# eniac/Reef

Hardware: AMD Instinct MI355X
Metric: msm_scalar_point_pairs_per_sec (higher is better)
Workload: dtype u32

## Files before the change

reef_amd/csrc/ec.h:

```cpp
#pragma once
#include "field.h"

#if defined(__HIP_DEVICE_COMPILE__)
#define REEF_ANY(x) __any(x)
#else
#define REEF_ANY(x) (x)
#endif

namespace reef {

struct affine {
    fe x, y;
};
struct xyzz {
    fe x, y, zz, zzz;
};
struct alignas(16) affine256 {
    fe256 x, y;
};
struct alignas(16) jacobian256 {
    fe256 x, y, z;
};
struct alignas(16) xyzz_mem {
    u32 w[36];
};

REEF_HD bool affine_is_inf(const affine &p) { return fe_is_literal_zero(p.x) && fe_is_literal_zero(p.y); }
template <int C> REEF_HD bool xyzz_is_inf(const xyzz &p) { return fe_is_zero<C>(p.zz); }

REEF_HD xyzz xyzz_identity() {
    xyzz r;
    r.x = fe_zero(); r.y = fe_zero(); r.zz = fe_zero(); r.zzz = fe_zero();
    return r;
}
REEF_HD xyzz xyzz_select(bool c, const xyzz &a, const xyzz &b) {
    xyzz r;
    r.x = fe_select(c, a.x, b.x); r.y = fe_select(c, a.y, b.y);
    r.zz = fe_select(c, a.zz, b.zz); r.zzz = fe_select(c, a.zzz, b.zzz);
    return r;
}
template <int C> REEF_HD xyzz xyzz_from_affine(const affine &p) {
    xyzz r;
    const bool inf = affine_is_inf(p);
    r.x = p.x; r.y = p.y;
    r.zz = fe_select(inf, fe_zero(), fe_one<C>());
    r.zzz = r.zz;
    return r;
}
template <int C> REEF_HD affine affine_neg(const affine &p) {
    affine r;
    r.x = p.x;
    r.y = fe_select(affine_is_inf(p), p.y, fe_neg<C, 2>(p.y));
    return r;
}
template <int C> REEF_HD xyzz xyzz_neg(const xyzz &p) {
    xyzz r = p;
    r.y = fe_neg<C, 4>(p.y);
    return r;
}

template <int C> REEF_HD xyzz xyzz_dbl_affine(const affine &p) {
    xyzz r;
    const fe u = fe_dbl<C>(p.y);
    const fe v = fe_sqr<C>(u);
    const fe w = fe_mul<C>(u, v);
    const fe s = fe_mul<C>(p.x, v);
    const fe xx = fe_sqr<C>(p.x);
    const fe m = fe_add<C>(fe_dbl<C>(xx), xx);
    r.x = fe_sub<C, 4>(fe_sqr<C>(m), fe_dbl<C>(s));
    r.y = fe_sub<C, 2>(fe_mul<C>(m, fe_sub<C, 8>(s, r.x)),
                       fe_mul<C>(w, p.y));
    r.zz = v;
    r.zzz = w;
    return r;
}

template <int C> REEF_HD xyzz xyzz_dbl(const xyzz &p) {
    xyzz r;
    const fe u = fe_dbl<C>(p.y);
    const fe v = fe_sqr<C>(u);
    const fe w = fe_mul<C>(u, v);
    const fe s = fe_mul<C>(p.x, v);
    const fe xx = fe_sqr<C>(p.x);
    const fe m = fe_add<C>(fe_dbl<C>(xx), xx);
    r.x = fe_sub<C, 4>(fe_sqr<C>(m), fe_dbl<C>(s));
    r.y = fe_sub<C, 2>(fe_mul<C>(m, fe_sub<C, 8>(s, r.x)),
                       fe_mul<C>(w, p.y));
    r.zz = fe_mul<C>(v, p.zz);
    r.zzz = fe_mul<C>(w, p.zzz);
    return r;
}

template <int C> REEF_HD xyzz xyzz_madd_flag(const xyzz &a, bool a_known_empty, const affine &p) {
    const bool a_inf = a_known_empty || xyzz_is_inf<C>(a);
    const bool p_inf = affine_is_inf(p);
    const fe pp_ = fe_mul_sub<C, 8>(p.x, a.zz, a.x);
    const fe rr = fe_mul_sub<C, 4>(p.y, a.zzz, a.y);
    xyzz r;
    if (__builtin_expect(fe_is_zero<C>(pp_) && fe_is_zero<C>(rr) && !a_inf && !p_inf, 0)) {
        r = xyzz_dbl_affine<C>(p);
    } else {
        const fe pp = fe_sqr<C>(pp_);
        const fe ppp = fe_mul<C>(pp_, pp);
        const fe q = fe_mul<C>(a.x, pp);
        fe t;
#pragma unroll
        for (int i = 0; i < 9; ++i) t.l[i] = ppp.l[i] + 2u * q.l[i];
        REEF_SET_BOUND(t, REEF_GET_BOUND(ppp) + 2.0 * REEF_GET_BOUND(q));
        r.x = fe_sqr_sub<C, 4>(rr, t);
        r.y = fe_mul2_add<C>(rr, fe_sub<C, 8>(q, r.x), fe_neg<C, 4>(a.y), ppp);
        r.zz = fe_mul<C>(a.zz, pp);
        r.zzz = fe_mul<C>(a.zzz, ppp);
    }
    if (REEF_ANY(a_inf)) {
        xyzz from_p;
        from_p.x = p.x; from_p.y = p.y; from_p.zz = fe_one<C>(); from_p.zzz = from_p.zz;
        r = xyzz_select(a_inf, from_p, r);
    }
    if (REEF_ANY(p_inf)) r = xyzz_select(p_inf, a, r);
    return r;
}

template <int C> REEF_HD xyzz xyzz_madd(const xyzz &a, const affine &p) { return xyzz_madd_flag<C>(a, false, p); }

template <int C> REEF_HD xyzz xyzz_add(const xyzz &a, const xyzz &b) {
    const bool a_inf = xyzz_is_inf<C>(a);
    const bool b_inf = xyzz_is_inf<C>(b);
    const fe u1 = fe_mul<C>(a.x, b.zz);
    const fe u2 = fe_mul<C>(b.x, a.zz);
    const fe s1 = fe_mul<C>(a.y, b.zzz);
    const fe s2 = fe_mul<C>(b.y, a.zzz);
    const fe pp_ = fe_sub<C, 2>(u2, u1);
    const fe rr = fe_sub<C, 2>(s2, s1);
    xyzz r;
    if (__builtin_expect(fe_is_zero<C>(pp_) && fe_is_zero<C>(rr) && !a_inf && !b_inf, 0)) {
        r = xyzz_dbl<C>(a);
    } else {
        const fe pp = fe_sqr<C>(pp_);
        const fe ppp = fe_mul<C>(pp_, pp);
        const fe q = fe_mul<C>(u1, pp);
        const fe t = fe_add<C>(ppp, fe_dbl<C>(q));
        r.x = fe_sub<C, 4>(fe_sqr<C>(rr), t);
        r.y = fe_mul2_add<C>(rr, fe_sub<C, 8>(q, r.x), fe_neg<C, 2>(s1), ppp);
        r.zz = fe_mul<C>(fe_mul<C>(a.zz, b.zz), pp);
        r.zzz = fe_mul<C>(fe_mul<C>(a.zzz, b.zzz), ppp);
    }
    r = xyzz_select(a_inf, b, r);
    r = xyzz_select(b_inf, a, r);
    return r;
}

REEF_HD affine affine_from_table(const affine256 &m) {
    affine r;
    r.x = fe_from_table(m.x);
    r.y = fe_from_table(m.y);
    return r;
}
template <int C> REEF_HD affine256 affine_to_table(const affine &p) {
    affine256 m;
    m.x = fe_to_table<C>(p.x);
    m.y = fe_to_table<C>(p.y);
    return m;
}
template <int C> REEF_HD affine affine_from_abi(const affine256 &m) {
    affine r;
    r.x = fe_from_abi<C>(m.x);
    r.y = fe_from_abi<C>(m.y);
    return r;
}
template <int C> REEF_HD affine256 affine_to_abi(const affine &p) {
    affine256 m;
    m.x = fe_to_abi<C>(p.x);
    m.y = fe_to_abi<C>(p.y);
    return m;
}
REEF_HD xyzz xyzz_from_mem(const xyzz_mem &m) {
    xyzz r;
#pragma unroll
    for (int i = 0; i < 9; ++i) {
        r.x.l[i] = m.w[i]; r.y.l[i] = m.w[9 + i]; r.zz.l[i] = m.w[18 + i]; r.zzz.l[i] = m.w[27 + i];
    }
    REEF_SET_BOUND(r.x, 6.0); REEF_SET_BOUND(r.y, 3.6); REEF_SET_BOUND(r.zz, 1.6); REEF_SET_BOUND(r.zzz, 1.6);
    return r;
}
REEF_HD xyzz_mem xyzz_to_mem(const xyzz &p) {
    xyzz_mem m;
#if defined(REEF_BOUNDS)
    if (p.x.bound > 6.0 || p.y.bound > 3.6 || p.zz.bound > 1.6 || p.zzz.bound > 1.6) REEF_BOUND_FAIL("xyzz_to_mem: invariant");
#endif
#pragma unroll
    for (int i = 0; i < 9; ++i) {
        m.w[i] = p.x.l[i]; m.w[9 + i] = p.y.l[i]; m.w[18 + i] = p.zz.l[i]; m.w[27 + i] = p.zzz.l[i];
    }
    return m;
}

template <int C> REEF_HD jacobian256 xyzz_to_abi_jacobian(const xyzz &p) {
    jacobian256 r;
    const bool inf = xyzz_is_inf<C>(p);
    r.x = fe_to_abi<C>(fe_select(inf, fe_zero(), fe_mul<C>(p.x, p.zz)));
    r.y = fe_to_abi<C>(fe_select(inf, fe_zero(), fe_mul<C>(p.y, p.zzz)));
    r.z = fe_to_abi<C>(fe_select(inf, fe_zero(), p.zz));
    return r;
}
template <int C> REEF_HD xyzz xyzz_from_abi_jacobian(const jacobian256 &m) {
    xyzz r;
    const fe z = fe_from_abi<C>(m.z);
    r.x = fe_from_abi<C>(m.x);
    r.y = fe_from_abi<C>(m.y);
    r.zz = fe_sqr<C>(z);
    r.zzz = fe_mul<C>(r.zz, z);
    return r;
}

template <int C> REEF_HD affine xyzz_to_affine_with_inv(const xyzz &p, const fe &t) {
    affine r;
    const bool inf = xyzz_is_inf<C>(p);
    const fe izz = fe_mul<C>(t, p.zzz);
    const fe izzz = fe_mul<C>(t, p.zz);
    r.x = fe_select(inf, fe_zero(), fe_mul<C>(p.x, izz));
    r.y = fe_select(inf, fe_zero(), fe_mul<C>(p.y, izzz));
    return r;
}
template <int C> REEF_HD affine xyzz_to_affine(const xyzz &p) {
    return xyzz_to_affine_with_inv<C>(p, fe_inv<C>(fe_mul<C>(p.zz, p.zzz)));
}

template <int C> REEF_HD fe256 affine_compress(const affine &p) {
    fe one = fe_zero();
    one.l[0] = 1;
    REEF_SET_BOUND(one, 1.0);
    fe256 x = fe_pack(fe_canon<C>(fe_mul<C>(p.x, one)));
    const fe y = fe_canon<C>(fe_mul<C>(p.y, one));
    x.w[7] |= (y.l[0] & 1u) << 31;
    if (affine_is_inf(p)) {
#pragma unroll
        for (int i = 0; i < 8; ++i) x.w[i] = 0;
    }
    return x;
}

template <int C> REEF_HD xyzz xyzz_scalar_mul(const affine &p, const u32 *k, int top_bit) {
    xyzz acc = xyzz_identity();
    for (int i = top_bit; i >= 0; --i) {
        acc = xyzz_dbl<C>(acc);
        if ((k[i >> 5] >> (i & 31)) & 1u) acc = xyzz_madd<C>(acc, p);
    }
    return acc;
}

}
```

reef_amd/csrc/field.h:

```cpp
#pragma once
#include <stdint.h>

#if defined(__HIPCC__)
#include <hip/hip_runtime.h>
#define REEF_HD __host__ __device__ __forceinline__
#else
#define REEF_HD inline
#endif

namespace reef {
typedef uint32_t u32;
typedef uint64_t u64;
typedef int64_t i64;
#if defined(__HIPCC__)
#if defined(REEF_VEC_VARIANT) && REEF_VEC_VARIANT == 2
typedef u32 u32x2 __attribute__((ext_vector_type(2), may_alias));
typedef u32 u32x4 __attribute__((ext_vector_type(4), may_alias));
REEF_HD u32x2 mk_u32x2(u32 a, u32 b) { u32x2 v; v.x = a; v.y = b; return v; }
REEF_HD u32x4 mk_u32x4(u32 a, u32 b, u32 c, u32 d) { u32x4 v; v.x = a; v.y = b; v.z = c; v.w = d; return v; }
#else
typedef uint2 u32x2;
typedef uint4 u32x4;
REEF_HD u32x2 mk_u32x2(u32 a, u32 b) { return make_uint2(a, b); }
REEF_HD u32x4 mk_u32x4(u32 a, u32 b, u32 c, u32 d) { return make_uint4(a, b, c, d); }
#endif
#endif
}

#include "field_consts.h"

#if defined(REEF_BOUNDS)
#include <assert.h>
#include <stdio.h>
#include <stdlib.h>
#define REEF_BOUND_FAIL(msg) do { fprintf(stderr, "REEF_BOUNDS violation: %s (%s:%d)\n", msg, __FILE__, __LINE__); abort(); } while (0)
#endif

namespace reef {

static constexpr u32 LIMB_BITS = 29;
static constexpr u32 LIMB_MASK = (1u << LIMB_BITS) - 1u;

struct fe {
    u32 l[9];
#if defined(REEF_BOUNDS)
    double bound;
#endif
};

struct alignas(16) fe256 {
    u32 w[8];
};

#if defined(REEF_BOUNDS)
#define REEF_SET_BOUND(x, b) ((x).bound = (b))
#define REEF_GET_BOUND(x) ((x).bound)
#else
#define REEF_SET_BOUND(x, b) ((void)0)
#define REEF_GET_BOUND(x) (0.0)
#endif

REEF_HD fe fe_zero() {
    fe r;
#pragma unroll
    for (int i = 0; i < 9; ++i) r.l[i] = 0;
    REEF_SET_BOUND(r, 0.0);
    return r;
}
template <int F> REEF_HD fe fe_const(const u32 (&c)[9], double bound) {
    fe r;
#pragma unroll
    for (int i = 0; i < 9; ++i) r.l[i] = c[i];
    REEF_SET_BOUND(r, bound);
    (void)bound;
    return r;
}
template <int F> REEF_HD fe fe_one() { return fe_const<F>(FC<F>::ONE, 1.0); }

REEF_HD fe fe_select(bool c, const fe &a, const fe &b) {
    fe r;
#pragma unroll
    for (int i = 0; i < 9; ++i) r.l[i] = c ? a.l[i] : b.l[i];
#if defined(REEF_BOUNDS)
    r.bound = a.bound > b.bound ? a.bound : b.bound;
#endif
    return r;
}

REEF_HD fe fe_norm(const fe &a) {
    fe r;
    r.l[0] = a.l[0] & LIMB_MASK;
#pragma unroll
    for (int i = 1; i < 8; ++i) r.l[i] = (a.l[i] & LIMB_MASK) + (a.l[i - 1] >> LIMB_BITS);
    r.l[8] = a.l[8] + (a.l[7] >> LIMB_BITS);
#if defined(REEF_BOUNDS)
    r.bound = a.bound;
    if ((u64)a.l[8] + (a.l[7] >> LIMB_BITS) >= (1ull << 29)) REEF_BOUND_FAIL("top limb overflow in fe_norm");
#endif
    return r;
}

REEF_HD fe fe_norm_strict(const fe &a) {
    fe r;
    u32 c = 0;
#pragma unroll
    for (int i = 0; i < 8; ++i) {
        u32 t = a.l[i] + c;
        r.l[i] = t & LIMB_MASK;
        c = t >> LIMB_BITS;
    }
    r.l[8] = a.l[8] + c;
#if defined(REEF_BOUNDS)
    r.bound = a.bound;
#endif
    return r;
}

template <int F> REEF_HD fe fe_add(const fe &a, const fe &b) {
    fe s;
#pragma unroll
    for (int i = 0; i < 9; ++i) s.l[i] = a.l[i] + b.l[i];
    REEF_SET_BOUND(s, REEF_GET_BOUND(a) + REEF_GET_BOUND(b));
    return fe_norm(s);
}
template <int F> REEF_HD fe fe_dbl(const fe &a) { return fe_add<F>(a, a); }

template <int F, int K> REEF_HD const u32 (&fe_bias())[9] {
    static_assert(K == 2 || K == 4 || K == 8 || K == 16 || K == 32, "bias");
    if constexpr (K == 2) return FC<F>::BIAS2;
    else if constexpr (K == 4) return FC<F>::BIAS4;
    else if constexpr (K == 8) return FC<F>::BIAS8;
    else if constexpr (K == 16) return FC<F>::BIAS16;
    else return FC<F>::BIAS32;
}

template <int F, int K> REEF_HD fe fe_sub(const fe &a, const fe &b) {
    fe d;
#pragma unroll
    for (int i = 0; i < 9; ++i) d.l[i] = a.l[i] + fe_bias<F, K>()[i] - b.l[i];
#if defined(REEF_BOUNDS)
    if (b.bound > (double)K * (1.0 - 1e-5)) REEF_BOUND_FAIL("fe_sub: subtrahend bound exceeds the bias");
    for (int i = 0; i < 9; ++i) {
        i64 t = (i64)a.l[i] + (i64)fe_bias<F, K>()[i] - (i64)b.l[i];
        if (t < 0 || t >= (1ll << 32)) REEF_BOUND_FAIL("fe_sub: limb out of range");
    }
    d.bound = a.bound + K;
#endif
    return fe_norm(d);
}
template <int F, int K> REEF_HD fe fe_neg(const fe &a) { return fe_sub<F, K>(fe_zero(), a); }

#if defined(__HIP_DEVICE_COMPILE__)
__device__ __forceinline__ void mad_acc_1(u64 &acc, u32 a) {
    u64 sink;
    asm("v_mad_u64_u32 %0, %1, %2, 1, %0" : "+v"(acc), "=&s"(sink) : "v"(a));
}
#else
REEF_HD void mad_acc_1(u64 &acc, u32 a) { acc += a; }
#endif

#if !defined(__HIP_DEVICE_COMPILE__)
REEF_HD void mad_row_new(u64 (&t)[10], const u32 (&a)[9], u32 b, u64 bias) {
    for (int j = 0; j < 9; ++j) t[j] = (u64)a[j] * b + bias;
}
REEF_HD void mad_row_acc(u64 (&t)[10], const u32 (&a)[9], u32 b) {
    for (int j = 0; j < 8; ++j) t[j] += (u64)a[j] * b;
    t[8] = (u64)a[8] * b;
}
REEF_HD void mad_row_add(u64 (&t)[10], const u32 (&a)[9], u32 b) {
    for (int j = 0; j < 9; ++j) t[j] += (u64)a[j] * b;
}
REEF_HD void mad_reduce(u64 (&t)[10], u32 q, u32 m1, u32 m2, u32 m3, u32 m4, u32 top) {
    t[1] += (u64)q * m1; t[2] += (u64)q * m2; t[3] += (u64)q * m3; t[4] += (u64)q * m4;
    t[8] += (u64)q * top;
}
template <int I> REEF_HD void sqr_row(u64 (&t)[10], const u32 (&a)[9], const u32 (&a2)[9], u64 bias) {
    if (I == 0) {
        t[0] = (u64)a[0] * a[0] + bias;
        for (int j = 1; j < 9; ++j) t[j] = (u64)a[0] * a2[j] + bias;
    } else if (I == 8) {
        t[8] = (u64)a[8] * a[8];
    } else {
        t[I] += (u64)a[I] * a[I];
        for (int j = I + 1; j < 8; ++j) t[j] += (u64)a[I] * a2[j];
        t[8] = (u64)a[I] * a2[8];
    }
}
#else
}
#include "field_mad_gfx950.h"
namespace reef {
template <int I> __device__ __forceinline__ void sqr_row(u64 (&t)[10], const u32 (&a)[9], const u32 (&a2)[9], u64 bias) {
    if constexpr (I == 0) sqr_row0(t, a, a2, bias);
    else if constexpr (I == 1) sqr_row1(t, a, a2);
    else if constexpr (I == 2) sqr_row2(t, a, a2);
    else if constexpr (I == 3) sqr_row3(t, a, a2);
    else if constexpr (I == 4) sqr_row4(t, a, a2);
    else if constexpr (I == 5) sqr_row5(t, a, a2);
    else if constexpr (I == 6) sqr_row6(t, a, a2);
    else if constexpr (I == 7) sqr_row7(t, a, a2);
    else sqr_row8(t, a, a2);
    (void)bias;
}
#endif

static constexpr u64 MONT_BIAS = LIMB_MASK;
REEF_HD void mont_bias(u64 (&t)[10]) {
#pragma unroll
    for (int j = 0; j < 9; ++j) t[j] += MONT_BIAS;
}

template <int F> REEF_HD void mont_round(u64 (&t)[10]) {
    const u32 q = ~(u32)t[0] & LIMB_MASK;
    mad_reduce(t, q, FC<F>::M1, FC<F>::M2, FC<F>::M3, FC<F>::M4, 1u << 22);
    t[1] += t[0] >> LIMB_BITS;
#pragma unroll
    for (int j = 0; j < 9; ++j) t[j] = t[j + 1];
}

template <int F> REEF_HD fe mont_finish(const u64 (&t)[10]) {
    fe r;
    u64 c = 0;
#pragma unroll
    for (int i = 0; i < 8; ++i) {
        const u64 v = t[i] + c;
        r.l[i] = (u32)v & LIMB_MASK;
        c = v >> LIMB_BITS;
    }
    r.l[8] = (u32)(t[8] + c);
#if defined(REEF_BOUNDS)
    if (t[8] + c >= (1ull << 29)) REEF_BOUND_FAIL("Montgomery product: result top limb overflow");
#endif
    return r;
}

template <int F> REEF_HD fe fe_mul(const fe &a, const fe &b) {
#if defined(REEF_BOUNDS)
    if (a.bound * b.bound >= 128.0) REEF_BOUND_FAIL("fe_mul: (A/M)(B/M) >= 128");
    for (int i = 0; i < 8; ++i)
        if (a.l[i] > LIMB_MASK + 8 || b.l[i] > LIMB_MASK + 8) REEF_BOUND_FAIL("fe_mul: operand not normalised");
#endif
    u64 t[10];
    t[9] = 0;
    mad_row_new(t, a.l, b.l[0], MONT_BIAS);
    mont_round<F>(t);
#pragma unroll
    for (int i = 1; i < 9; ++i) {
        mad_row_acc(t, a.l, b.l[i]);
        mont_round<F>(t);
    }
    fe r = mont_finish<F>(t);
    REEF_SET_BOUND(r, 1.0 + REEF_GET_BOUND(a) * REEF_GET_BOUND(b) / 128.0);
    return r;
}

template <int F> REEF_HD fe fe_mul2_add(const fe &a, const fe &b, const fe &c, const fe &d) {
#if defined(REEF_BOUNDS)
    if (a.bound * b.bound + c.bound * d.bound >= 128.0) REEF_BOUND_FAIL("fe_mul2_add: (A/M)(B/M) + (C/M)(D/M) >= 128");
    for (int i = 0; i < 8; ++i)
        if (a.l[i] > LIMB_MASK + 8 || b.l[i] > LIMB_MASK + 8 || c.l[i] > LIMB_MASK + 8 || d.l[i] > LIMB_MASK + 8)
            REEF_BOUND_FAIL("fe_mul2_add: operand not normalised");
#endif
    u64 t[10];
    t[9] = 0;
    mad_row_new(t, a.l, b.l[0], MONT_BIAS);
    mad_row_add(t, c.l, d.l[0]);
    mont_round<F>(t);
#pragma unroll
    for (int i = 1; i < 9; ++i) {
        mad_row_acc(t, a.l, b.l[i]);
        mad_row_add(t, c.l, d.l[i]);
        mont_round<F>(t);
    }
    fe r = mont_finish<F>(t);
    REEF_SET_BOUND(r, 1.0 + (REEF_GET_BOUND(a) * REEF_GET_BOUND(b) + REEF_GET_BOUND(c) * REEF_GET_BOUND(d)) / 128.0);
    return r;
}

template <int F, int K> REEF_HD fe fe_mul_sub(const fe &a, const fe &b, const fe &c) {
#if defined(REEF_BOUNDS)
    if (a.bound * b.bound >= 128.0) REEF_BOUND_FAIL("fe_mul_sub: (A/M)(B/M) >= 128");
    if (c.bound > (double)K * (1.0 - 1e-5)) REEF_BOUND_FAIL("fe_mul_sub: subtrahend bound exceeds the bias");
    for (int i = 0; i < 8; ++i)
        if (a.l[i] > LIMB_MASK + 8 || b.l[i] > LIMB_MASK + 8) REEF_BOUND_FAIL("fe_mul_sub: operand not normalised");
    for (int i = 0; i < 9; ++i)
        if (c.l[i] > fe_bias<F, K>()[i]) REEF_BOUND_FAIL("fe_mul_sub: subtrahend limb exceeds the bias limb");
#endif
    u64 t[10];
    t[9] = 0;
    mad_row_new(t, a.l, b.l[0], MONT_BIAS);
    mont_round<F>(t);
#pragma unroll
    for (int i = 1; i < 9; ++i) {
        mad_row_acc(t, a.l, b.l[i]);
        mont_round<F>(t);
    }
#pragma unroll
    for (int i = 0; i < 9; ++i) mad_acc_1(t[i], fe_bias<F, K>()[i] - c.l[i]);
    fe r = mont_finish<F>(t);
    REEF_SET_BOUND(r, 1.0 + REEF_GET_BOUND(a) * REEF_GET_BOUND(b) / 128.0 + K);
    return r;
}

template <int F> REEF_HD fe fe_sqr(const fe &a) {
#if defined(REEF_BOUNDS)
    if (a.bound * a.bound >= 128.0) REEF_BOUND_FAIL("fe_sqr: (A/M)^2 >= 128");
    for (int i = 0; i < 8; ++i)
        if (a.l[i] > LIMB_MASK + 8) REEF_BOUND_FAIL("fe_sqr: operand not normalised");
#endif
    u32 a2[9];
#pragma unroll
    for (int i = 0; i < 9; ++i) a2[i] = a.l[i] << 1;
    u64 t[10];
    t[9] = 0;
    sqr_row<0>(t, a.l, a2, MONT_BIAS); mont_round<F>(t);
    sqr_row<1>(t, a.l, a2, MONT_BIAS); mont_round<F>(t);
    sqr_row<2>(t, a.l, a2, MONT_BIAS); mont_round<F>(t);
    sqr_row<3>(t, a.l, a2, MONT_BIAS); mont_round<F>(t);
    sqr_row<4>(t, a.l, a2, MONT_BIAS); mont_round<F>(t);
    sqr_row<5>(t, a.l, a2, MONT_BIAS); mont_round<F>(t);
    sqr_row<6>(t, a.l, a2, MONT_BIAS); mont_round<F>(t);
    sqr_row<7>(t, a.l, a2, MONT_BIAS); mont_round<F>(t);
    sqr_row<8>(t, a.l, a2, MONT_BIAS); mont_round<F>(t);
    fe r = mont_finish<F>(t);
    REEF_SET_BOUND(r, 1.0 + REEF_GET_BOUND(a) * REEF_GET_BOUND(a) / 128.0);
    return r;
}

template <int F, int K> REEF_HD fe fe_sqr_sub(const fe &a, const fe &c) {
#if defined(REEF_BOUNDS)
    if (a.bound * a.bound >= 128.0) REEF_BOUND_FAIL("fe_sqr_sub: (A/M)^2 >= 128");
    if (c.bound > (double)K * (1.0 - 1e-5)) REEF_BOUND_FAIL("fe_sqr_sub: subtrahend bound exceeds the bias");
    for (int i = 0; i < 8; ++i)
        if (a.l[i] > LIMB_MASK + 8) REEF_BOUND_FAIL("fe_sqr_sub: operand not normalised");
    for (int i = 0; i < 9; ++i)
        if (c.l[i] > fe_bias<F, K>()[i]) REEF_BOUND_FAIL("fe_sqr_sub: subtrahend limb exceeds the bias limb");
#endif
    u32 a2[9];
#pragma unroll
    for (int i = 0; i < 9; ++i) a2[i] = a.l[i] << 1;
    u64 t[10];
    t[9] = 0;
    sqr_row<0>(t, a.l, a2, MONT_BIAS); mont_round<F>(t);
    sqr_row<1>(t, a.l, a2, MONT_BIAS); mont_round<F>(t);
    sqr_row<2>(t, a.l, a2, MONT_BIAS); mont_round<F>(t);
    sqr_row<3>(t, a.l, a2, MONT_BIAS); mont_round<F>(t);
    sqr_row<4>(t, a.l, a2, MONT_BIAS); mont_round<F>(t);
    sqr_row<5>(t, a.l, a2, MONT_BIAS); mont_round<F>(t);
    sqr_row<6>(t, a.l, a2, MONT_BIAS); mont_round<F>(t);
    sqr_row<7>(t, a.l, a2, MONT_BIAS); mont_round<F>(t);
    sqr_row<8>(t, a.l, a2, MONT_BIAS); mont_round<F>(t);
#pragma unroll
    for (int i = 0; i < 9; ++i) mad_acc_1(t[i], fe_bias<F, K>()[i] - c.l[i]);
    fe r = mont_finish<F>(t);
    REEF_SET_BOUND(r, 1.0 + REEF_GET_BOUND(a) * REEF_GET_BOUND(a) / 128.0 + K);
    return r;
}

template <int F> REEF_HD fe fe_small_multiple(u32 j) {
    fe r;
    u64 c = 0;
#pragma unroll
    for (int i = 0; i < 8; ++i) {
        u64 v = (u64)j * FC<F>::MOD[i] + c;
        r.l[i] = (u32)v & LIMB_MASK;
        c = v >> LIMB_BITS;
    }
    r.l[8] = (u32)((u64)j * FC<F>::MOD[8] + c);
    REEF_SET_BOUND(r, (double)j);
    return r;
}

template <int F> REEF_HD bool fe_is_zero(const fe &a) {
#if defined(REEF_BOUNDS)
    if (a.bound >= 64.0) REEF_BOUND_FAIL("fe_is_zero: bound >= 64");
#endif
    const u32 j = a.l[0];
    if (__builtin_expect(j >= 64u, 1)) return false;
    const fe s = fe_norm_strict(a);
    const fe m = fe_small_multiple<F>(j);
    u32 d = 0;
#pragma unroll
    for (int i = 0; i < 9; ++i) d |= s.l[i] ^ m.l[i];
    return d == 0;
}
REEF_HD bool fe_is_literal_zero(const fe &a) {
    u32 d = 0;
#pragma unroll
    for (int i = 0; i < 9; ++i) d |= a.l[i];
    return d == 0;
}

template <int F> REEF_HD fe fe_canon(const fe &a) {
    const fe s = fe_norm_strict(a);
    const u32 q = s.l[8] >> 22;
    fe r;
    i64 c = 0;
#pragma unroll
    for (int i = 0; i < 8; ++i) {
        i64 v = (i64)s.l[i] - (i64)((u64)q * FC<F>::MOD[i]) + c;
        r.l[i] = (u32)v & LIMB_MASK;
        c = v >> LIMB_BITS;
    }
    i64 top = (i64)s.l[8] - (i64)((u64)q * FC<F>::MOD[8]) + c;
    const bool neg = top < 0;
    u32 cc = 0;
#pragma unroll
    for (int i = 0; i < 8; ++i) {
        u32 v = r.l[i] + (neg ? FC<F>::MOD[i] : 0u) + cc;
        r.l[i] = v & LIMB_MASK;
        cc = v >> LIMB_BITS;
    }
    r.l[8] = (u32)(top + (neg ? (i64)FC<F>::MOD[8] : 0) + cc);
    REEF_SET_BOUND(r, 1.0);
    return r;
}

REEF_HD fe fe_unpack(const fe256 &p) {
    fe r;
#pragma unroll
    for (int i = 0; i < 9; ++i) {
        const int bit = 29 * i, w = bit >> 5, s = bit & 31;
        u32 v = p.w[w] >> s;
        if (s > 3 && w + 1 < 8) v |= p.w[w + 1] << (32 - s);
        r.l[i] = (i == 8) ? v : (v & LIMB_MASK);
    }
    REEF_SET_BOUND(r, 4.0);
    return r;
}
REEF_HD fe256 fe_pack(const fe &a) {
    fe256 p;
#pragma unroll
    for (int w = 0; w < 8; ++w) {
        const int bit = 32 * w, i = bit / 29, s = bit - 29 * i;
        u32 v = a.l[i] >> s;
        if (i + 1 < 9) v |= a.l[i + 1] << (29 - s);
        if (29 - s + 29 < 32 && i + 2 < 9) v |= a.l[i + 2] << (58 - s);
        p.w[w] = v;
    }
    return p;
}

template <int F> REEF_HD fe fe_from_abi(const fe256 &p) {
    fe x = fe_unpack(p);
    REEF_SET_BOUND(x, 1.0);
    return fe_mul<F>(x, fe_const<F>(FC<F>::C_IN, 1.0));
}
template <int F> REEF_HD fe256 fe_to_abi(const fe &a) {
    return fe_pack(fe_canon<F>(fe_mul<F>(a, fe_const<F>(FC<F>::C_OUT, 1.0))));
}
template <int F> REEF_HD fe256 fe_to_table(const fe &a) { return fe_pack(fe_canon<F>(a)); }
REEF_HD fe fe_from_table(const fe256 &p) {
    fe x = fe_unpack(p);
    REEF_SET_BOUND(x, 1.0);
    return x;
}
template <int F> REEF_HD fe256 fe_abi_to_integer(const fe256 &p) {
    fe x = fe_unpack(p);
    REEF_SET_BOUND(x, 1.0);
    fe c32 = fe_zero();
    c32.l[0] = 32;
    REEF_SET_BOUND(c32, 1.0);
    return fe_pack(fe_canon<F>(fe_mul<F>(x, c32)));
}
template <int F> REEF_HD fe fe_from_integer(const fe256 &p) {
    fe x = fe_unpack(p);
    REEF_SET_BOUND(x, 1.0);
    return fe_mul<F>(x, fe_const<F>(FC<F>::C_R2, 1.0));
}
template <int F> REEF_HD fe256 fe_to_integer(const fe &x) {
    fe one = fe_zero();
    one.l[0] = 1;
    REEF_SET_BOUND(one, 1.0);
    return fe_pack(fe_canon<F>(fe_mul<F>(x, one)));
}
template <int F> REEF_HD fe fe_from_caller(const fe256 &p, bool is_mont) { return is_mont ? fe_from_abi<F>(p) : fe_from_integer<F>(p); }
template <int F> REEF_HD fe256 fe_to_caller(const fe &x, bool to_mont) { return to_mont ? fe_to_abi<F>(x) : fe_to_integer<F>(x); }

template <int F> REEF_HD fe fe_inv(const fe &a) {
    u32 e[9];
#pragma unroll
    for (int i = 0; i < 9; ++i) e[i] = FC<F>::MOD[i];
    e[0] = LIMB_MASK;
    e[1] -= 1;
    fe acc = fe_one<F>();
    for (int i = 254; i >= 0; --i) {
        acc = fe_sqr<F>(acc);
        const int limb = i / 29, bit = i - 29 * limb;
        if ((e[limb] >> bit) & 1u) acc = fe_mul<F>(acc, a);
    }
    return acc;
}

}
```

reef_amd/csrc/msm_kernels.inc:

```
#include "ec.h"
#include "ec_coop.h"
#include "glv_consts.h"

namespace reef {

static constexpr u32 KEY_INVALID = 0xffffffffu;
static constexpr int WAVE = 64;

template <int C> struct Kern;

__device__ __forceinline__ void latency_critical() { __builtin_amdgcn_s_setprio(3); }

__device__ __forceinline__ u32 extract_bits(const fe256 &k, u32 off, u32 c) {
    const u32 limb = off >> 5, sh = off & 31u;
    u32 lo = 0, hi = 0;
#pragma unroll
    for (u32 l = 0; l < 8; ++l) {
        lo = (l == limb) ? k.w[l] : lo;
        hi = (l == limb + 1) ? k.w[l] : hi;
    }
    u64 v = (((u64)hi << 32) | lo) >> sh;
    return (u32)v & ((1u << c) - 1u);
}

// ... 398 lines not shown
    for (u32 k = threadIdx.x; k < fine; k += blockDim.x) hist[k] = 0;
    __syncthreads();
    for (u32 e = e0 + threadIdx.x; e < e1; e += 4 * blockDim.x) {
        u32 k[4];
#pragma unroll
        for (int u = 0; u < 4; ++u) {
            k[u] = 0xffffffffu;
            if (e + u * blockDim.x < e1) {
                if constexpr (COMPACT) k[u] = static_cast<const u32 *>(in_)[e + u * blockDim.x];
                else k[u] = static_cast<const u32x2 *>(in_)[e + u * blockDim.x].x;
            }
        }
#pragma unroll
        for (int u = 0; u < 4; ++u)
            if (e + u * blockDim.x < e1) atomicAdd(&hist[k[u] & (fine - 1u)], 1u);
    }
    __syncthreads();
    for (u32 k = threadIdx.x; k < fine; k += blockDim.x) seg_counts[(size_t)blockIdx.x * fine + k] = hist[k];
}

static __global__ void __launch_bounds__(1024) k_fine_offsets(const u32 *__restrict__ bin_start, const u32 *__restrict__ seg_first, u32 nbins,
                                                      u32 shift, u32 *__restrict__ seg_counts, u32 *__restrict__ bucket_start) {
    latency_critical();
    __shared__ u32 lds[192];
    const u32 bin = blockIdx.x, f = threadIdx.x, fine = 1u << shift;
    const u32 s0 = seg_first[bin], s1 = seg_first[bin + 1];
    u32 tot = 0;
    for (u32 sg = s0; sg < s1; ++sg) tot += seg_counts[(size_t)sg * fine + f];
    u32 total;
    const u32 ex = block_exclusive_scan(tot, lds, total);
    u32 run = bin_start[bin] + ex;
    bucket_start[(size_t)bin * fine + f] = run;
    for (u32 sg = s0; sg < s1; ++sg) {
        u32 *p = seg_counts + (size_t)sg * fine + f;
        const u32 t = *p;
        *p = run;
        run += t;
    }
    if (bin == 0 && f == 0) bucket_start[(size_t)nbins * fine] = bin_start[nbins];
}

template <bool COMPACT, bool WORD = false>
static __global__ void __launch_bounds__(1024) k_fine_scatter(const void *__restrict__ in_, const u32 *__restrict__ bin_start,
                                                      const u32 *__restrict__ seg_first, u32 nbins, u32 shift,
                                                      const u32 *__restrict__ seg_cursors, void *__restrict__ out_) {
    latency_critical();
    extern __shared__ u32 cur[];
    const u32 fine = 1u << shift;
    u32 bin, e0, e1;
    if (!seg_lookup(bin_start, seg_first, nbins, blockIdx.x, bin, e0, e1)) return;
    for (u32 k = threadIdx.x; k < fine; k += blockDim.x) cur[k] = seg_cursors[(size_t)blockIdx.x * fine + k];
    __syncthreads();
    for (u32 e = e0 + threadIdx.x; e < e1; e += 4 * blockDim.x) {
        u32x2 v[4];
#pragma unroll
        for (int u = 0; u < 4; ++u) {
            v[u] = mk_u32x2(0, 0);
            if (e + u * blockDim.x < e1) {
                if constexpr (COMPACT) {
                    const u32 w = static_cast<const u32 *>(in_)[e + u * blockDim.x];
                    v[u] = mk_u32x2((bin << shift) | (w & (fine - 1u)), ((w & 0x7fffffffu) >> shift) | (w & 0x80000000u));
                } else {
                    v[u] = static_cast<const u32x2 *>(in_)[e + u * blockDim.x];
                }
            }
        }
#pragma unroll
        for (int u = 0; u < 4; ++u)
            if (e + u * blockDim.x < e1) {
                const u32 pos = atomicAdd(&cur[v[u].x & (fine - 1u)], 1u);
                if constexpr (WORD) static_cast<u32 *>(out_)[pos] = v[u].y;
                else static_cast<u32x2 *>(out_)[pos] = v[u];
            }
    }
}

struct RowSortShape {
    u32 rows, row_len;
    u32 W, G, NB;
    u32 rows_per_block;
    u32 n_ctx, L0;
};

static __global__ void __launch_bounds__(1024) k_row_count(const u32 *__restrict__ dig, RowSortShape sh, u32 *__restrict__ counts) {
    latency_critical();
    extern __shared__ u32 hist[];
    const u32 r0 = blockIdx.x * sh.rows_per_block;
    const u32 nrows = min(sh.rows_per_block, sh.rows - r0);
    const u32 nkeys = nrows * sh.G * sh.NB;
    for (u32 k = threadIdx.x; k < nkeys; k += blockDim.x) hist[k] = 0;
    __syncthreads();
    const size_t n = (size_t)sh.rows * sh.row_len;
    const u32 cnt = nrows * sh.row_len;
    for (u32 w = 0; w < sh.W; ++w) {
        const u32 *d = dig + (size_t)w * n + (size_t)r0 * sh.row_len;
        const u32 g = w % sh.G;
        for (u32 e = threadIdx.x; e < cnt; e += blockDim.x) {
            const u32 mag = d[e] & 0x7fffffffu;
            if (mag) atomicAdd(&hist[((e / sh.row_len) * sh.G + g) * sh.NB + mag - 1u], 1u);
        }
    }
    __syncthreads();
    u32 *out = counts + (size_t)r0 * sh.G * sh.NB;
    for (u32 k = threadIdx.x; k < nkeys; k += blockDim.x) out[k] = hist[k];
}

static __global__ void __launch_bounds__(1024) k_row_scatter(const u32 *__restrict__ dig, RowSortShape sh,
                                                     const u32 *__restrict__ bucket_start, u32x2 *__restrict__ entries) {
    latency_critical();
    extern __shared__ u32 cur[];
    const u32 r0 = blockIdx.x * sh.rows_per_block;
    const u32 nrows = min(sh.rows_per_block, sh.rows - r0);
    const u32 nkeys = nrows * sh.G * sh.NB;
    const u32 key0 = r0 * sh.G * sh.NB;
    for (u32 k = threadIdx.x; k < nkeys; k += blockDim.x) cur[k] = bucket_start[key0 + k];
    __syncthreads();
    const size_t n = (size_t)sh.rows * sh.row_len;
    const u32 cnt = nrows * sh.row_len;
    for (u32 w = 0; w < sh.W; ++w) {
        const u32 *d = dig + (size_t)w * n + (size_t)r0 * sh.row_len;
        const u32 g = w % sh.G, j = w / sh.G;
        for (u32 e = threadIdx.x; e < cnt; e += blockDim.x) {
            const u32 v = d[e];
            const u32 mag = v & 0x7fffffffu;
            if (mag) {
                const u32 row = e / sh.row_len, col = e - row * sh.row_len;
                const u32 rel = (row * sh.G + g) * sh.NB + mag - 1u;
                const u32 pos = atomicAdd(&cur[rel], 1u);
                entries[pos] = mk_u32x2(key0 + rel, (j * sh.n_ctx + col) | (v & 0x80000000u));
            }
        }
    }
}

template <int C, bool COOP>
__device__ __forceinline__ void merge_wave(u32 ka, u32 kb, xyzz v, xyzz bv, u32 wave_id, int lane, int role, CoopLds *L,
                                           xyzz_mem *__restrict__ bucket_acc, u32 *__restrict__ out_keys, xyzz_mem *__restrict__ out_vals);


__device__ __forceinline__ u32 bucket_of(const u32 *__restrict__ bs, u32 nbt, u32 p) {
    u32 lo = 0, hi = nbt;
    while (hi - lo > 1) {
        const u32 mid = (lo + hi) >> 1;
        if (bs[mid] <= p) lo = mid; else hi = mid;
    }
    return lo;
}
template <int C, bool FUSED, bool WORD = false>
__global__ void __launch_bounds__(256) k_accum0(const affine256 *__restrict__ tables, const void *__restrict__ entries_,
                                               const u32 *__restrict__ m_ptr, u32 L0,
                                               u32 nchunks, xyzz_mem *__restrict__ bucket_acc, u32 *__restrict__ out_keys,
                                               xyzz_mem *__restrict__ out_vals, u32 nbt = 0) {
    __shared__ xyzz_mem stash[FUSED ? 256 : 1];
    const u32 t = blockIdx.x * blockDim.x + threadIdx.x;
    if constexpr (FUSED) {
        if (((t >> 6) << 6) >= nchunks) return;
    } else {
        if (t >= nchunks) return;
    }
    const u32 M = *m_ptr;
    while (L0 > 8 && (u64)(L0 >> 1) * nchunks >= M) L0 >>= 1;
    const u32 start = t * L0;
    u32 key_a = KEY_INVALID, key_b = KEY_INVALID;
    xyzz tail = xyzz_identity();
    if (t < nchunks && start < M) {
        const u32 end = min(start + L0, M);
        const u32 cnt = end - start;
        const u32x2 *mine = static_cast<const u32x2 *>(entries_) + start;
        const u32 *mine1 = static_cast<const u32 *>(entries_) + start;
        const u32 *bs = m_ptr - nbt;
        u32 cur_key, pay, boundary = 0;
        bool lo_open, ro_open = false;
        u32 prev_key = KEY_INVALID, next_key = KEY_INVALID;
        if constexpr (WORD) {
            cur_key = bucket_of(bs, nbt, start);
            boundary = bs[cur_key + 1];
            lo_open = bs[cur_key] < start;
            pay = mine1[0];
        } else {
            prev_key = start > 0 ? static_cast<const u32x2 *>(entries_)[start - 1].x : KEY_INVALID;
            next_key = end < M ? static_cast<const u32x2 *>(entries_)[end].x : KEY_INVALID;
            const u32x2 e0 = mine[0];
            cur_key = e0.x;
            pay = e0.y;
            lo_open = prev_key == cur_key;
        }
        affine256 raw = load_affine256(tables + (pay & 0x7fffffffu));
        xyzz acc = xyzz_identity();
        bool acc_empty = true;
        bool first_run = true;
        for (u32 k = 0; k < cnt; ++k) {
            u32 nkey = cur_key, npay = 0;
            affine256 nraw = raw;
            if (k + 1 < cnt) {
                if constexpr (WORD) {
                    npay = mine1[k + 1];
                    if (start + k + 1 == boundary) {
                        nkey = cur_key + 1;
                        if (bs[nkey + 1] == boundary) nkey = bucket_of(bs, nbt, boundary);
                    }
                } else {
                    const u32x2 e = mine[k + 1];
                    nkey = e.x;
                    npay = e.y;
                }
                nraw = load_affine256(tables + (npay & 0x7fffffffu));
            }
            affine pt = affine_from_table(raw);
            pt.y = fe_select((pay >> 31) != 0 && !affine_is_inf(pt), fe_neg<C, 2>(pt.y), pt.y);
            acc = xyzz_madd_flag<C>(acc, acc_empty, pt);
            acc_empty = false;
            const bool last = (k + 1 == cnt);
            if (last || nkey != cur_key) {
                const bool lo = first_run && lo_open;
                bool ro;
                if constexpr (WORD) ro = last && boundary > end;
                else ro = last && next_key == cur_key;
                if (!lo && !ro) {
                    store_xyzz(bucket_acc + cur_key, acc);
                } else if (lo) {
                    if constexpr (FUSED) store_xyzz(&stash[threadIdx.x], acc);
                    else store_xyzz(out_vals + 2 * (size_t)t, acc);
                    key_a = cur_key;
                    if (ro) {
                        if constexpr (!FUSED) store_xyzz(out_vals + 2 * (size_t)t + 1, xyzz_identity());
                        key_b = cur_key;
                    }
                } else {
                    if constexpr (FUSED) tail = acc;
                    else store_xyzz(out_vals + 2 * (size_t)t + 1, acc);
                    key_b = cur_key;
                }
                first_run = false;
                acc = xyzz_identity();
                acc_empty = true;
                if constexpr (WORD) { if (!last) boundary = bs[nkey + 1]; }
            }
            cur_key = nkey; pay = npay; raw = nraw;
        }
        (void)ro_open; (void)prev_key;
    }
    if constexpr (FUSED) {
        latency_critical();
        xyzz v = xyzz_identity();
        if (key_a != KEY_INVALID) v = load_xyzz(&stash[threadIdx.x]);
        merge_wave<C, false>(key_a, key_b, v, tail, t >> 6, (int)(threadIdx.x & 63), 0, nullptr, bucket_acc, out_keys, out_vals);
    } else {
        out_keys[2 * (size_t)t] = key_a;
        out_keys[2 * (size_t)t + 1] = key_b;
    }
}

template <int C>
__global__ void __launch_bounds__(256) k_accumN(const u32 *__restrict__ in_keys, const xyzz_mem *__restrict__ in_vals,
                                               u32 len, xyzz_mem *__restrict__ bucket_acc, u32 *__restrict__ out_keys,
                                               xyzz_mem *__restrict__ out_vals) {
    latency_critical();
    const u32 gid = blockIdx.x * blockDim.x + threadIdx.x;
    const int lane = threadIdx.x & 63;
    const u32 wave_id = gid >> 6;
    const u32 wave_first = gid - lane;
    if (wave_first >= len) return;
    const u32 key = gid < len ? in_keys[gid] : KEY_INVALID;
    const bool valid = key != KEY_INVALID;
    if (!__any(valid)) {
        if (lane == 0) { out_keys[2 * (size_t)wave_id] = KEY_INVALID; out_keys[2 * (size_t)wave_id + 1] = KEY_INVALID; }
        return;
    }
    xyzz v = xyzz_identity();
    if (valid) v = load_xyzz(in_vals + gid);
    for (int d = 1; d < 64; d <<= 1) {
        const u32 pk = __shfl_down(key, d, WAVE);
        const bool need = valid && (lane + d < 64) && pk == key;
        if (__any(need)) {
            xyzz o = shfl_xyzz(v, (lane + d) & 63);
            xyzz s = xyzz_add<C>(v, o);
            v = xyzz_select(need, s, v);
        }
    }
    const u32 key_up = __shfl_up(key, 1, WAVE);
    const bool is_head = valid && (lane == 0 || key_up != key);
    const u32 key63 = __shfl(key, 63, WAVE);
    const u32 prev_key = wave_first > 0 ? in_keys[wave_first - 1] : KEY_INVALID;
    const u32 next_key = wave_first + 64 < len ? in_keys[wave_first + 64] : KEY_INVALID;
    if (is_head) {
        const bool lo = (lane == 0) && prev_key == key;
        const bool ro = (key63 == key) && next_key == key;
        if (!lo && !ro) {
            store_xyzz(bucket_acc + key, v);
        } else if (lo) {
            store_xyzz(out_vals + 2 * (size_t)wave_id, v);
            if (ro) store_xyzz(out_vals + 2 * (size_t)wave_id + 1, xyzz_identity());
        } else {
            store_xyzz(out_vals + 2 * (size_t)wave_id + 1, v);
        }
    }
    if (lane == 0) {
        out_keys[2 * (size_t)wave_id] = (valid && prev_key == key) ? key : KEY_INVALID;
        out_keys[2 * (size_t)wave_id + 1] = (key63 != KEY_INVALID && next_key == key63) ? key63 : KEY_INVALID;
    }
}

template <int C, bool COOP>
__device__ __forceinline__ void merge_wave(u32 ka, u32 kb, xyzz v, xyzz bv, u32 wave_id, int lane, int role, CoopLds *L,
                                           xyzz_mem *__restrict__ bucket_acc, u32 *__restrict__ out_keys, xyzz_mem *__restrict__ out_vals) {
    const bool has_a = ka != KEY_INVALID;
    const bool interior = has_a && kb == ka;
    const bool has_b = kb != KEY_INVALID && !interior;
    if (!__any(has_a || has_b)) {
        if (lane == 0 && (!COOP || role == 0)) { out_keys[2 * (size_t)wave_id] = KEY_INVALID; out_keys[2 * (size_t)wave_id + 1] = KEY_INVALID; }
        return;
    }
    const int b_before = __shfl_up(has_b ? 1 : 0, 1, WAVE);
    const bool recv = lane > 0 && b_before != 0;
    for (int step = 0; step < 7; ++step) {
        const int d = step == 0 ? 63 : 1 << (step - 1);
        const u32 ka_d = __shfl(ka, (lane + d) & 63, WAVE);
        bool need;
        if (step == 0) need = recv;
        else need = has_a && lane + d < 64 && ka_d == ka;
        if (__any(need)) {
            const xyzz o = shfl_xyzz(step == 0 ? bv : v, (lane + d) & 63);
            xyzz sum;
            if constexpr (COOP) sum = xyzz_add_coop<C>(v, o, *L, role, lane);
            else sum = xyzz_add<C>(v, o);
            v = xyzz_select(need, sum, v);
        }
    }
    const u32 ka_up = __shfl_up(ka, 1, WAVE);
    const bool is_head = has_a && (lane == 0 || ka_up != ka);
    const u32 ka63 = __shfl(ka, 63, WAVE);
    const bool interior63 = __shfl(interior ? 1 : 0, 63, WAVE) != 0;
    const bool hasb63 = __shfl(has_b ? 1 : 0, 63, WAVE) != 0;
    const u32 kb63 = __shfl(kb, 63, WAVE);
    const u32 ka0 = __shfl(ka, 0, WAVE);
    if (COOP && role != 0) return;
    if (is_head) {
        const bool lo = lane == 0;
        const bool ro = interior63 && ka63 == ka;
        if (!lo && !ro) {
            store_xyzz(bucket_acc + ka, v);
        } else if (lo) {
            store_xyzz(out_vals + 2 * (size_t)wave_id, v);
            if (ro) store_xyzz(out_vals + 2 * (size_t)wave_id + 1, xyzz_identity());
        } else {
            store_xyzz(out_vals + 2 * (size_t)wave_id + 1, v);
        }
    }
    if (lane == 63 && has_b) store_xyzz(out_vals + 2 * (size_t)wave_id + 1, bv);
    if (lane == 0) {
        out_keys[2 * (size_t)wave_id] = ka0;
        out_keys[2 * (size_t)wave_id + 1] = interior63 ? ka63 : (hasb63 ? kb63 : KEY_INVALID);
    }
}

template <int C, bool COOP>
__global__ void __launch_bounds__(256) k_merge_chunks(const u32 *__restrict__ in_keys, const xyzz_mem *__restrict__ in_vals, u32 nchunks,
                                                     xyzz_mem *__restrict__ bucket_acc, u32 *__restrict__ out_keys, xyzz_mem *__restrict__ out_vals) {
    latency_critical();
    __shared__ CoopLds L;
    const int lane = threadIdx.x & 63, role = threadIdx.x >> 6;
    const u32 wave_id = COOP ? blockIdx.x : blockIdx.x * 4u + (u32)role;
    const u32 first = wave_id * 64u;
    if (first >= nchunks) return;
    const u32 t = first + lane;
    const bool in_range = t < nchunks;
    const u32 ka = in_range ? in_keys[2 * (size_t)t] : KEY_INVALID;
    const u32 kb = in_range ? in_keys[2 * (size_t)t + 1] : KEY_INVALID;
    const bool has_a = ka != KEY_INVALID;
    const bool has_b = kb != KEY_INVALID && !(has_a && kb == ka);
    xyzz v = xyzz_identity(), bv = xyzz_identity();
    if (has_a) v = load_xyzz_coop(in_vals + 2 * (size_t)t);
    if (has_b) bv = load_xyzz_coop(in_vals + 2 * (size_t)t + 1);
    merge_wave<C, COOP>(ka, kb, v, bv, wave_id, lane, role, &L, bucket_acc, out_keys, out_vals);
}

template <int C, int LPS>
__global__ void __launch_bounds__(256) k_reduce_rowcol(const xyzz_mem *__restrict__ bucket_acc,
                                                      const u32 *__restrict__ bucket_start, u32 c1, u32 c2, u32 groups,
                                                      xyzz_mem *__restrict__ rowcol) {
    static_assert(LPS == 64 || LPS == 32 || LPS == 16, "lanes per sum");
    latency_critical();
    constexpr u32 SPW = 64 / LPS;
    const u32 rows = 1u << c1, cols = 1u << c2, per_group = rows + cols, sums = groups * per_group;
    const u32 wave = (blockIdx.x * blockDim.x + threadIdx.x) >> 6;
    const int lane = threadIdx.x & 63, l = lane & (LPS - 1);
    if (wave * SPW >= sums) return;
    const u32 sum = wave * SPW + (u32)lane / LPS;
    const bool valid = sum < sums;
    const u32 g = sum / per_group, idx = sum - g * per_group;
    const bool is_row = idx < rows;
// ... 1396 lines not shown
```

Before: 930.0 million.

## Restructure bucket-accumulate loop to cut register pressure in mixed addition

The mixed-add routine now always runs the generic addition formula and applies the doubling, identity and infinity cases afterwards in one rare wave-uniform branch. When the point is infinity, the accumulator is saved to shared memory rather than kept live in registers. Point negation is done on the packed 256-bit table form through a conditional subtraction from 2p, and the prefetch loop is unrolled by two with ping-pong buffers so the per-iteration register copies go away. The aim is lower VGPR use and fewer divergent branches, paid for with an extra shared-memory array, a looser y bound and more complicated special-case handling.

```diff
diff --git a/reef_amd/csrc/ec.h b/reef_amd/csrc/ec.h
--- a/reef_amd/csrc/ec.h
+++ b/reef_amd/csrc/ec.h
@@ -91,34 +91,43 @@
     return r;
 }
 
-template <int C> REEF_HD xyzz xyzz_madd_flag(const xyzz &a, bool a_known_empty, const affine &p) {
+REEF_HD xyzz xyzz_from_mem(const xyzz_mem &m);
+REEF_HD xyzz_mem xyzz_to_mem(const xyzz &p);
+
+template <int C> REEF_HD xyzz xyzz_madd_flag(const xyzz &a, bool a_known_empty, const affine &p, bool p_inf, xyzz_mem *keep) {
     const bool a_inf = a_known_empty || xyzz_is_inf<C>(a);
-    const bool p_inf = affine_is_inf(p);
+    if (__builtin_expect(REEF_ANY(p_inf), 0)) {
+        if (p_inf) *keep = xyzz_to_mem(a);
+    }
     const fe pp_ = fe_mul_sub<C, 8>(p.x, a.zz, a.x);
     const fe rr = fe_mul_sub<C, 4>(p.y, a.zzz, a.y);
     xyzz r;
-    if (__builtin_expect(fe_is_zero<C>(pp_) && fe_is_zero<C>(rr) && !a_inf && !p_inf, 0)) {
-        r = xyzz_dbl_affine<C>(p);
-    } else {
-        const fe pp = fe_sqr<C>(pp_);
-        const fe ppp = fe_mul<C>(pp_, pp);
-        const fe q = fe_mul<C>(a.x, pp);
-        fe t;
-#pragma unroll
-        for (int i = 0; i < 9; ++i) t.l[i] = ppp.l[i] + 2u * q.l[i];
-        REEF_SET_BOUND(t, REEF_GET_BOUND(ppp) + 2.0 * REEF_GET_BOUND(q));
-        r.x = fe_sqr_sub<C, 4>(rr, t);
-        r.y = fe_mul2_add<C>(rr, fe_sub<C, 8>(q, r.x), fe_neg<C, 4>(a.y), ppp);
-        r.zz = fe_mul<C>(a.zz, pp);
-        r.zzz = fe_mul<C>(a.zzz, ppp);
-    }
-    if (REEF_ANY(a_inf)) {
-        xyzz from_p;
-        from_p.x = p.x; from_p.y = p.y; from_p.zz = fe_one<C>(); from_p.zzz = from_p.zz;
-        r = xyzz_select(a_inf, from_p, r);
-    }
-    if (REEF_ANY(p_inf)) r = xyzz_select(p_inf, a, r);
-    return r;
+    const fe pp = fe_sqr<C>(pp_);
+    const fe ppp = fe_mul<C>(pp_, pp);
+    const fe q = fe_mul<C>(a.x, pp);
+    fe t;
+#pragma unroll
+    for (int i = 0; i < 9; ++i) t.l[i] = ppp.l[i] + 2u * q.l[i];
+    REEF_SET_BOUND(t, REEF_GET_BOUND(ppp) + 2.0 * REEF_GET_BOUND(q));
+    r.x = fe_sqr_sub<C, 4>(rr, t);
+    r.y = fe_mul2_add<C>(rr, fe_sub<C, 8>(q, r.x), fe_neg<C, 4>(a.y), ppp);
+    r.zz = fe_mul<C>(a.zz, pp);
+    r.zzz = fe_mul<C>(a.zzz, ppp);
+    const bool dbl = fe_is_zero<C>(pp_) && fe_is_zero<C>(rr) && !a_inf && !p_inf;
+    if (__builtin_expect(REEF_ANY(a_inf || p_inf || dbl), 0)) {
+        xyzz alt;
+        alt.x = p.x; alt.y = p.y; alt.zz = fe_one<C>(); alt.zzz = alt.zz;
+        if (REEF_ANY(dbl)) alt = xyzz_select(dbl, xyzz_dbl_affine<C>(p), alt);
+        if (REEF_ANY(p_inf)) {
+            if (p_inf) alt = xyzz_from_mem(*keep);
+        }
+        r = xyzz_select(a_inf || p_inf || dbl, alt, r);
+    }
+    return r;
+}
+template <int C> REEF_HD xyzz xyzz_madd_flag(const xyzz &a, bool a_known_empty, const affine &p) {
+    xyzz_mem keep;
+    return xyzz_madd_flag<C>(a, a_known_empty, p, affine_is_inf(p), &keep);
 }
 
 template <int C> REEF_HD xyzz xyzz_madd(const xyzz &a, const affine &p) { return xyzz_madd_flag<C>(a, false, p); }
@@ -156,6 +165,17 @@
     r.y = fe_from_table(m.y);
     return r;
 }
+template <int C> REEF_HD affine affine_from_table_signed(const affine256 &m, bool neg, bool &inf) {
+    u32 d = 0;
+#pragma unroll
+    for (int i = 0; i < 8; ++i) d |= m.x.w[i] | m.y.w[i];
+    inf = d == 0;
+    const bool n = neg && !inf;
+    affine r;
+    r.x = fe_from_table(m.x);
+    r.y = fe_from_table_signed(fe_neg_if<C>(m.y, n), n);
+    return r;
+}
 template <int C> REEF_HD affine256 affine_to_table(const affine &p) {
     affine256 m;
     m.x = fe_to_table<C>(p.x);
diff --git a/reef_amd/csrc/field.h b/reef_amd/csrc/field.h
--- a/reef_amd/csrc/field.h
+++ b/reef_amd/csrc/field.h
@@ -149,7 +149,6 @@
     return fe_norm(d);
 }
 template <int F, int K> REEF_HD fe fe_neg(const fe &a) { return fe_sub<F, K>(fe_zero(), a); }
-
 #if defined(__HIP_DEVICE_COMPILE__)
 __device__ __forceinline__ void mad_acc_1(u64 &acc, u32 a) {
     u64 sink;
@@ -455,6 +454,39 @@
     REEF_SET_BOUND(x, 1.0);
     return x;
 }
+template <int F> constexpr fe256 fe_two_m_packed() {
+    fe256 r = {};
+    for (int i = 0; i < 9; ++i) {
+        const int bit = 29 * i;
+        u64 v = ((u64)FC<F>::MOD[i] * 2u) << (bit & 31);
+        for (int j = bit >> 5; j < 8 && v != 0; ++j) {
+            const u64 t = (u64)r.w[j] + (v & 0xffffffffu);
+            r.w[j] = (u32)t;
+            v = (v >> 32) + (t >> 32);
+        }
+    }
+    return r;
+}
+template <int F> REEF_HD fe256 fe_neg_if(const fe256 &a, bool neg) {
+    constexpr fe256 c = fe_two_m_packed<F>();
+    fe256 r;
+    u32 borrow = 0;
+#pragma unroll
+    for (int i = 0; i < 8; ++i) {
+        u32 d, e;
+        const u32 b1 = __builtin_usub_overflow(c.w[i], a.w[i], &d);
+        const u32 b2 = __builtin_usub_overflow(d, borrow, &e);
+        r.w[i] = neg ? e : a.w[i];
+        borrow = b1 | b2;
+    }
+    return r;
+}
+REEF_HD fe fe_from_table_signed(const fe256 &p, bool neg) {
+    fe x = fe_unpack(p);
+    REEF_SET_BOUND(x, neg ? 2.0 : 1.0);
+    (void)neg;
+    return x;
+}
 template <int F> REEF_HD fe256 fe_abi_to_integer(const fe256 &p) {
     fe x = fe_unpack(p);
     REEF_SET_BOUND(x, 1.0);
diff --git a/reef_amd/csrc/msm_kernels.inc b/reef_amd/csrc/msm_kernels.inc
--- a/reef_amd/csrc/msm_kernels.inc
+++ b/reef_amd/csrc/msm_kernels.inc
@@ -574,6 +574,7 @@
                                                u32 nchunks, xyzz_mem *__restrict__ bucket_acc, u32 *__restrict__ out_keys,
                                                xyzz_mem *__restrict__ out_vals, u32 nbt = 0) {
     __shared__ xyzz_mem stash[FUSED ? 256 : 1];
+    __shared__ xyzz_mem keep[256];
     const u32 t = blockIdx.x * blockDim.x + threadIdx.x;
     if constexpr (FUSED) {
         if (((t >> 6) << 6) >= nchunks) return;
@@ -607,58 +608,66 @@
             pay = e0.y;
             lo_open = prev_key == cur_key;
         }
-        affine256 raw = load_affine256(tables + (pay & 0x7fffffffu));
         xyzz acc = xyzz_identity();
         bool acc_empty = true;
         bool first_run = true;
-        for (u32 k = 0; k < cnt; ++k) {
-            u32 nkey = cur_key, npay = 0;
-            affine256 nraw = raw;
-            if (k + 1 < cnt) {
-                if constexpr (WORD) {
-                    npay = mine1[k + 1];
-                    if (start + k + 1 == boundary) {
-                        nkey = cur_key + 1;
-                        if (bs[nkey + 1] == boundary) nkey = bucket_of(bs, nbt, boundary);
-                    }
-                } else {
-                    const u32x2 e = mine[k + 1];
-                    nkey = e.x;
-                    npay = e.y;
+        auto fetch = [&](u32 k1, u32 ckey, u32 &nkey, u32 &npay, affine256 &nraw) {
+            nkey = ckey;
+            if constexpr (WORD) {
+                npay = mine1[k1];
+                if (start + k1 == boundary) {
+                    nkey = ckey + 1;
+                    if (bs[nkey + 1] == boundary) nkey = bucket_of(bs, nbt, boundary);
                 }
-                nraw = load_affine256(tables + (npay & 0x7fffffffu));
+            } else {
+                const u32x2 e = mine[k1];
+                nkey = e.x;
+                npay = e.y;
             }
-            affine pt = affine_from_table(raw);
-            pt.y = fe_select((pay >> 31) != 0 && !affine_is_inf(pt), fe_neg<C, 2>(pt.y), pt.y);
-            acc = xyzz_madd_flag<C>(acc, acc_empty, pt);
+            nraw = load_affine256(tables + (npay & 0x7fffffffu));
+        };
+        auto add_entry = [&](u32 k, u32 ckey, u32 cpay, const affine256 &craw, u32 nkey) {
+            bool p_inf;
+            const affine pt = affine_from_table_signed<C>(craw, (cpay >> 31) != 0, p_inf);
+            acc = xyzz_madd_flag<C>(acc, acc_empty, pt, p_inf, &keep[threadIdx.x]);
             acc_empty = false;
             const bool last = (k + 1 == cnt);
-            if (last || nkey != cur_key) {
+            if (last || nkey != ckey) {
                 const bool lo = first_run && lo_open;
                 bool ro;
                 if constexpr (WORD) ro = last && boundary > end;
-                else ro = last && next_key == cur_key;
+                else ro = last && next_key == ckey;
                 if (!lo && !ro) {
-                    store_xyzz(bucket_acc + cur_key, acc);
+                    store_xyzz(bucket_acc + ckey, acc);
                 } else if (lo) {
                     if constexpr (FUSED) store_xyzz(&stash[threadIdx.x], acc);
                     else store_xyzz(out_vals + 2 * (size_t)t, acc);
-                    key_a = cur_key;
+                    key_a = ckey;
                     if (ro) {
                         if constexpr (!FUSED) store_xyzz(out_vals + 2 * (size_t)t + 1, xyzz_identity());
-                        key_b = cur_key;
+                        key_b = ckey;
                     }
                 } else {
                     if constexpr (FUSED) tail = acc;
                     else store_xyzz(out_vals + 2 * (size_t)t + 1, acc);
-                    key_b = cur_key;
+                    key_b = ckey;
                 }
                 first_run = false;
                 acc = xyzz_identity();
                 acc_empty = true;
                 if constexpr (WORD) { if (!last) boundary = bs[nkey + 1]; }
             }
-            cur_key = nkey; pay = npay; raw = nraw;
+        };
+        u32 key0 = cur_key, pay0 = pay, key1 = cur_key, pay1 = 0;
+        affine256 raw0 = load_affine256(tables + (pay0 & 0x7fffffffu));
+        affine256 raw1 = raw0;
+        for (u32 k = 0; k < cnt; k += 2) {
+            if (k + 1 < cnt) fetch(k + 1, key0, key1, pay1, raw1);
+            add_entry(k, key0, pay0, raw0, key1);
+            if (k + 1 < cnt) {
+                if (k + 2 < cnt) fetch(k + 2, key1, key0, pay0, raw0);
+                add_entry(k + 1, key1, pay1, raw1, key0);
+            }
         }
         (void)ro_open; (void)prev_key;
     }
```

New measurement: 928.0 million. No clear change (-0.2%).
